# BjarkeHautop/bayesSSM

Measured on AMD Instinct MI355X. Metric: particle-steps/sec (N x T), bootstrap filter, higher is better.
Workload: dtype f64; 1 GPU; BASELINE C2: linear-Gaussian SSM, bootstrap filter, T=1000, N=1048576, SISR + systematic resampling, return_particles=FALSE, device generator; per_gpu=one independent filter replica per GPU (no data-path collective), backend=single process

## Files before the change

bayesssm_amd/csrc/fused.hip.h:

```cpp
#pragma once
#include "kernels.hip.h"

namespace bssm {

typedef unsigned long long fz_u64;
#define BSSM_RLX_AGENT __ATOMIC_RELAXED, __HIP_MEMORY_SCOPE_AGENT

constexpr int FZ_MAXB = 2 * NT;
constexpr int FZ_MINB = 256;
constexpr int FZ_KREC = 8;
constexpr int FZ_KSIDE = (int)(sizeof(SideEntry) / 4);
constexpr int FZ_NREP = 16;
constexpr int FZ_MAXSIDE = 16;
constexpr uint32_t FLAG_FUSED_BAIL = 8u, FLAG_FUSED_TIMEOUT = 16u;
constexpr uint32_t FZ_ST_DOIT = 1u, FZ_ST_DEAD = 2u, FZ_ST_STOP = 4u, FZ_ST_BAIL = 8u;
constexpr long long FZ_TIMEOUT_TICKS = 2000000ll;

struct FusedWs {
    fz_u64 e1[6][FZ_MAXB];
    fz_u64 c1[FZ_NREP][16];
    fz_u64 a1[2][FZ_MAXB];
    fz_u64 e2[FZ_KREC][FZ_MAXB];
    fz_u64 c2[FZ_NREP][16];
    fz_u64 e3[FZ_KREC][FZ_MAXB];
    fz_u64 c3[FZ_NREP][16];
    fz_u64 a3[2][FZ_MAXB];
    fz_u64 side_w[FZ_MAXB][FZ_MAXSIDE][FZ_KSIDE];
    fz_u64 side_p[FZ_MAXB][FZ_MAXSIDE][FZ_KSIDE];
    BlockRec brec_priv[2][MAXB];
    SideList side_priv[2][FZ_MAXB];
    long long stamps[2][24];
    long long startt[FZ_MAXB];
    long long endt[FZ_MAXB];
    long long waket[3][FZ_MAXB];
    long long pubt[4][FZ_MAXB];
};

#ifdef BSSM_DEV_STAMPS
#define FZ_STAMP(k) do { if (fz_stamper) g.ws->stamps[fz_row][k] = clock64(); } while (0)
#else
#define FZ_STAMP(k) do { } while (0)
#endif

__device__ __forceinline__ fz_u64 fz_gran(uint32_t tag, uint32_t v) { return ((fz_u64)tag << 32) | v; }
__device__ __forceinline__ void fz_put(fz_u64* g, uint32_t tag, uint32_t v) { __hip_atomic_store(g, fz_gran(tag, v), BSSM_RLX_AGENT); }
__device__ __forceinline__ void fz_put64(fz_u64* g, uint32_t tag, uint64_t v) { fz_put(g, tag, (uint32_t)v); fz_put(g + 1, tag, (uint32_t)(v >> 32)); }
__device__ __forceinline__ void fz_put64x(fz_u64* g, int stride, uint32_t tag, uint64_t v) { fz_put(g, tag, (uint32_t)v); fz_put(g + stride, tag, (uint32_t)(v >> 32)); }
__device__ __forceinline__ fz_u64 fz_get(const fz_u64* g) { return __hip_atomic_load(g, BSSM_RLX_AGENT); }

__device__ __forceinline__ void fz_encode(const BlockRec& br, uint32_t (&w)[FZ_KREC])
{
    const Rec& r = br.prefix;
    const long long d1 = (long long)(r.o[1] - r.o[0]), d2 = (long long)(r.o[2] - r.o[0]), d3 = (long long)(r.o[3] - r.o[0]);
    const bool fits = d1 >= -32768 && d1 <= 32767 && d2 >= -32768 && d2 <= 32767 && d3 >= -32768 && d3 <= 32767;
    const uint32_t meta = (uint32_t)(r.kind & 3) | ((uint32_t)(br.nside & 127) << 2) | ((br.tail_from < NT) ? (1u << 9) : 0u) | (fits ? 0u : (1u << 10));
    w[0] = (uint32_t)r.base; w[1] = (uint32_t)(r.base >> 32); w[2] = (uint32_t)r.o[0]; w[3] = (uint32_t)(r.o[0] >> 32);
    w[4] = ((uint32_t)d1 & 0xffffu) | (((uint32_t)d2 & 0xffffu) << 16);
    w[5] = ((uint32_t)d3 & 0xffffu) | (meta << 16);
    w[6] = (uint32_t)r.lo; w[7] = (uint32_t)r.hi;
}
__device__ __forceinline__ BlockRec fz_decode(const uint32_t (&w)[FZ_KREC], bool& unsupported)
{
    BlockRec br;
    Rec& r = br.prefix;
    r.base = mk64(w[0], w[1]); r.o[0] = mk64(w[2], w[3]);
    r.o[1] = r.o[0] + (uint64_t)(long long)(int16_t)(w[4] & 0xffffu);
    r.o[2] = r.o[0] + (uint64_t)(long long)(int16_t)(w[4] >> 16);
    r.o[3] = r.o[0] + (uint64_t)(long long)(int16_t)(w[5] & 0xffffu);
    const uint32_t meta = w[5] >> 16;
    r.kind = (int32_t)(meta & 3); r.lo = (int32_t)w[6]; r.hi = (int32_t)w[7]; r.pad = 0;
    br.nside = (int32_t)((meta >> 2) & 127);
    const bool tail = (meta >> 9) & 1u, unenc = (meta >> 10) & 1u;
    br.tail_from = tail ? 0 : NT;
    unsupported = tail || unenc || br.nside > FZ_MAXSIDE;
    return br;
}

struct FzClock { long long t0; __device__ __forceinline__ bool expired() const { return (long long)wall_clock64() - t0 > FZ_TIMEOUT_TICKS; } };

template <int NG>
__device__ __forceinline__ bool fz_wait_slot(const fz_u64* slot, uint32_t tag, const FzClock& clk, uint32_t& val)
{
    const int lane = threadIdx.x & 63;
    for (unsigned spins = 0;; spins++) {
        bool ok = true;
        if (lane < NG) { const fz_u64 x = fz_get(slot + lane); ok = (uint32_t)(x >> 32) == tag; val = (uint32_t)x; }
        if (__all(ok)) return true;
        if ((spins & 31u) == 31u && clk.expired()) return false;
        __builtin_amdgcn_s_sleep(1);
    }
}

template <int NG>
__device__ __forceinline__ bool fz_wait_words(const fz_u64* mine, uint32_t tag, const FzClock& clk, uint32_t& val)
{
    const int lane = threadIdx.x & 63;
    for (unsigned spins = 0;; spins++) {
        bool ok = true;
        if (lane < NG) { const fz_u64 x = fz_get(mine); ok = (uint32_t)(x >> 32) == tag; val = (uint32_t)x; }
        if (__all(ok)) return true;
        if ((spins & 31u) == 31u && clk.expired()) return false;
        __builtin_amdgcn_s_sleep(1);
    }
}

struct LaneTerms { double a[EL]; };
__device__ __attribute__((noinline)) void fz_block_literal(uint64_t* tin , uint64_t cin, double* terms , const LaneTerms v ,
                                                           DevState* st)
{
    const int t = threadIdx.x;
#pragma unroll
    for (int k = 0; k < EL; k++) terms[t * EL + k] = v.a[k];
    __syncthreads();
    if (t == 0) {
        double c = b2d(cin);
        for (int tt = 0; tt < NT; tt++) {
            tin[tt] = d2b(c);
            for (int k = 0; k < EL; k++) c = c + terms[tt * EL + k];
        }
        atomicAdd((unsigned long long*)&st->stat_serial_walks, 1ull);
        atomicAdd((unsigned long long*)&st->stat_literal_terms, (unsigned long long)EB);
    }
    __syncthreads();
}
__device__ __forceinline__ LaneTerms fz_lane_terms(const double (&v)[EL])
{
    LaneTerms r;
#pragma unroll
    for (int k = 0; k < EL; k++) r.a[k] = v[k];
    return r;
}

struct FusedRecSink {
    fz_u64* rec_planes;
    fz_u64* side_base;
    int bidx; uint32_t tag;
    double* terms; DevState* st;
    __device__ __forceinline__ void rec(const BlockRec& br) const
    {
        uint32_t w[FZ_KREC];
        fz_encode(br, w);
#pragma unroll
        for (int k = 0; k < FZ_KREC; k++) fz_put(rec_planes + (size_t)k * FZ_MAXB + bidx, tag, w[k]);
    }
    __device__ __forceinline__ void side(int k, const SideEntry& e) const
    {
        if (k >= FZ_MAXSIDE) return;
        uint32_t w[FZ_KSIDE];
        memcpy(w, &e, sizeof(SideEntry));
        fz_u64* dst = side_base + ((size_t)bidx * FZ_MAXSIDE + k) * FZ_KSIDE;
#pragma unroll
        for (int q = 0; q < FZ_KSIDE; q++) fz_put(dst + q, tag, w[q]);
    }
    __device__ __forceinline__ void literal(uint64_t* tin, uint64_t cin, const double (&v)[EL]) const { fz_block_literal(tin, cin, terms, fz_lane_terms(v), st); }
};

struct FusedArgs {
    const double* xin;
    long long N; int nblk;
    ModelPar par; double y; NoiseSrc ns; int trans;
    int obs_i, resample_algorithm; double threshold;
    double* ess_out; double* llh_out; int* resampled_out;
    double* w_out;
    int lim;
    int force_fallback;
    ApplyArgs a;
    FusedWs* ws; uint32_t tag;
    double* znext; uint32_t znext_call;
};

struct FusedSmem {
    double red[16]; double redq[16];
    uint32_t slot[16];
    int bail;
    double bm, bs_, bq;
};

template <int NG>
__device__ __forceinline__ bool fz_gather(const fz_u64* planes, int c0, int c1, uint32_t tag, const FzClock& clk, int* bail, uint32_t (&w0)[NG], uint32_t (&w1)[NG])
{
    const bool pair = ((c0 & 1) == 0) && (c0 < c1);
    const bool want1 = (c0 + 1 < c1);
    __amdgpu_buffer_rsrc_t rs = __builtin_amdgcn_make_buffer_rsrc((void*)const_cast<fz_u64*>(planes), 0, NG * FZ_MAXB * 8, 0x00020000);
    bool have = false;
    for (unsigned spins = 0;; spins++) {
        if (!have) {
            bool ok = true;
            if (pair) {
#pragma unroll
                for (int k = 0; k < NG; k++) {
                    const u32x4_t x = __builtin_amdgcn_raw_buffer_load_b128(rs, (k * FZ_MAXB + c0) * 8, 0, 16);
                    ok = ok && x.y == tag && (!want1 || x.w == tag); w0[k] = x.x; w1[k] = x.z;
                }
            } else {
#pragma unroll
                for (int k = 0; k < NG; k++) {
                    if (c0 < c1) { const fz_u64 x = fz_get(planes + (size_t)k * FZ_MAXB + c0); ok = ok && (uint32_t)(x >> 32) == tag; w0[k] = (uint32_t)x; }
                    if (c0 + 1 < c1) { const fz_u64 x = fz_get(planes + (size_t)k * FZ_MAXB + c0 + 1); ok = ok && (uint32_t)(x >> 32) == tag; w1[k] = (uint32_t)x; }
                }
            }
            have = ok;
        }
        if (__all(have)) return true;
        if ((spins & 15u) == 15u && clk.expired()) { *bail = 1; return false; }
        if (*(volatile int*)bail) return false;
        __builtin_amdgcn_s_sleep(1);
    }
}

__device__ __forceinline__ bool fz_fetch_sides(const fz_u64* side_base, SideList* side_priv, int b, int nside, uint32_t tag, const FzClock& clk)
{
    for (int k = 0; k < nside; k++) {
        const fz_u64* src = side_base + ((size_t)b * FZ_MAXSIDE + k) * FZ_KSIDE;
        uint32_t w[FZ_KSIDE];
        for (unsigned spins = 0;; spins++) {
            bool ok = true;
#pragma unroll
            for (int q = 0; q < FZ_KSIDE; q++) { const fz_u64 x = fz_get(src + q); ok = ok && (uint32_t)(x >> 32) == tag; w[q] = (uint32_t)x; }
            if (ok) break;
            if ((spins & 15u) == 15u && clk.expired()) return false;
            __builtin_amdgcn_s_sleep(1);
        }
        SideEntry e;
        memcpy(&e, w, sizeof(SideEntry));
        side_priv[b].e[k] = e;
    }
    return true;
}

struct FzLateSide {
    static constexpr bool active = true;
    const fz_u64* src; uint32_t tag; FzClock clk;
    __device__ __forceinline__ unsigned long long issue() const
    {
        const int lane = threadIdx.x & 63;
        static_assert(FZ_KSIDE <= 64, "one granule per lane");
        return (lane < FZ_KSIDE) ? fz_get(src + lane) : 0ull;
    }
    __device__ __forceinline__ bool finish(SideEntry* dst, unsigned long long x) const
    {
        const int lane = threadIdx.x & 63;
        for (unsigned spins = 0;; spins++) {
            const bool ok = (lane >= FZ_KSIDE) || ((uint32_t)(x >> 32) == tag);
            if (__all(ok)) {
                if (lane < FZ_KSIDE) reinterpret_cast<uint32_t*>(dst)[lane] = (uint32_t)x;
                __builtin_amdgcn_fence(__ATOMIC_RELEASE, "wavefront");
                __builtin_amdgcn_wave_barrier();
                __builtin_amdgcn_fence(__ATOMIC_ACQUIRE, "wavefront");
                return true;
            }
            if ((spins & 15u) == 15u && clk.expired()) return false;
            __builtin_amdgcn_s_sleep(1);
            if (lane < FZ_KSIDE) x = fz_get(src + lane);
        }
    }
};

template <int MODE, bool EMIT>
__device__ __forceinline__ uint64_t fz_resolve_duty(SegSmem& sm, ResolveSmem& rs, FusedSmem& fs, const FusedArgs& g, DevState* st, const FzClock& clk,
                                                    uint64_t* cin_lds , bool& bail)
{
    const int t = threadIdx.x, B = g.nblk;
    const fz_u64* planes = (MODE == MODE_W) ? &g.ws->e2[0][0] : &g.ws->e3[0][0];
    const fz_u64* sides = (MODE == MODE_W) ? &g.ws->side_w[0][0][0] : &g.ws->side_p[0][0][0];
    const int CB = (B + NT - 1) / NT;
    const int Bneed = (MODE == MODE_P) ? B - 1 : B;
    const int c0 = t * CB, c1 = (c0 + CB < Bneed) ? c0 + CB : Bneed;
    uint32_t w0[FZ_KREC], w1[FZ_KREC];
    bool ok = fz_gather<FZ_KREC>(planes, c0, c1, g.tag, clk, &fs.bail, w0, w1);
    bool unsup = false;
    BlockRec q0, q1;
    q0.prefix = rec_identity(0); q0.tail_from = NT; q0.nside = 0; q1 = q0;
    if (ok) {
        if (c0 < c1) {
            bool u; q0 = fz_decode(w0, u); unsup = unsup || u;
            if (!u && q0.nside > 0 && !(c0 == B - 1 && q0.nside == 1 && q0.tail_from >= NT)) {
#ifdef BSSM_DEV_STAMPS
                g.ws->pubt[3][20 + MODE] = c0; atomicAdd((unsigned long long*)&g.ws->pubt[3][22 + MODE], 1ull);
#endif
                ok = ok && fz_fetch_sides(sides, g.ws->side_priv[MODE], c0, q0.nside, g.tag, clk);
            }
        }
        if (c0 + 1 < c1) {
            bool u; q1 = fz_decode(w1, u); unsup = unsup || u;
            if (!u && q1.nside > 0 && !(c0 + 1 == B - 1 && q1.nside == 1 && q1.tail_from >= NT)) {
#ifdef BSSM_DEV_STAMPS
                g.ws->pubt[3][20 + MODE] = c0 + 1; atomicAdd((unsigned long long*)&g.ws->pubt[3][22 + MODE], 1ull);
#endif
                ok = ok && fz_fetch_sides(sides, g.ws->side_priv[MODE], c0 + 1, q1.nside, g.tag, clk);
            }
        }
    }
    if (unsup) atomicMax(&fs.bail, 2); else if (!ok) atomicMax(&fs.bail, 1);
    __syncthreads();
#ifdef BSSM_DEV_STAMPS
    if (t == 0) { g.ws->stamps[1][MODE == MODE_W ? 8 : 13] = clock64(); g.ws->pubt[3][8 + (MODE == MODE_W ? 1 : 2)] = (long long)wall_clock64(); }
#endif
    if (fs.bail) { bail = true; return 0ull; }
    long long lit = 0;
    const int upto = (MODE == MODE_P) ? B - 1 : B;
    FzLateSide late; late.src = sides + ((size_t)(B - 1) * FZ_MAXSIDE + 0) * FZ_KSIDE; late.tag = g.tag; late.clk = clk;
    const uint64_t fin = resolve_in_block<MODE, NT, EMIT, FzLateSide>(sm, rs, g.ws->brec_priv[MODE], g.ws->side_priv[MODE], B, upto, g.xin, g.N, 1.0, st, true, g.force_fallback, cin_lds, &lit, &q0, &q1, late);
    if (EMIT && t == 0) cin_lds[B - 1] = fin;
    if (lit >= LIT_FROM_W) fs.bail = 2;
    __syncthreads();
#ifdef BSSM_DEV_STAMPS
    if (t == 0) g.ws->stamps[1][MODE == MODE_W ? 9 : 14] = clock64();
#endif
    if (fs.bail) { bail = true; return 0ull; }
    return fin;
}

__host__ __device__ __forceinline__ int fz_resolver_block(int B) { return (5 * B) / 16; }

__device__ __forceinline__ void fz_draw_next(const FusedArgs& g, long long j0, long long N, const int prio_after = 1)
{
    if (!g.znext) return;
    __builtin_amdgcn_s_setprio(0);
#pragma unroll
    for (int i = 0; i < EL / 2; i++) {
        const long long j = j0 + 2 * i;
        if (j < N) {
            double z0, z1;
            normal_pair(g.ns.key, g.ns.purpose, g.znext_call, 0, (uint32_t)(j >> 1), z0, z1);
            if (j + 1 < N) bulk_store16<1>(g.znext + j, z0, z1);
            else g.znext[j] = z0;
        }
    }
    if (prio_after == 3) __builtin_amdgcn_s_setprio(3); else __builtin_amdgcn_s_setprio(1);
}

template <int MODEL, int KIND>
__global__ __launch_bounds__(NT) void k_obs(FusedArgs g, DevState* st)
{
    __shared__ SegSmem sm;
    __shared__ uint64_t tin[NT + 1];
    __shared__ FusedSmem fs;
    __shared__ int Tbegin;
    extern __shared__ __attribute__((aligned(16))) double dyn[];
    int* Tl = reinterpret_cast<int*>(dyn);
    double* lx = dyn + EB / 2;
    const int t = threadIdx.x, lane = t & 63, wave = t >> 6;
    const int bidx = (int)blockIdx.x, B = g.nblk;
    const bool resolver = (bidx == fz_resolver_block(B));
    if (resolver) __builtin_amdgcn_s_setprio(3); else __builtin_amdgcn_s_setprio(1);
    const bool fz_stamper = (t == 0) && (resolver || bidx == ((B > 100) ? 100 : 0)); const int fz_row = resolver ? 1 : 0; (void)fz_stamper; (void)fz_row;
    FZ_STAMP(0);
#ifdef BSSM_DEV_STAMPS
    if (t == 0) g.ws->startt[bidx] = (long long)wall_clock64();
#define FZ_PUBT(k) do { if (t == 0) g.ws->pubt[k][bidx] = (long long)wall_clock64(); } while (0)
#define FZ_GDONE(k) do { if (t == 0) g.ws->pubt[3][8 + (k)] = (long long)wall_clock64(); } while (0)
#define FZ_WAKE(k) do { if (t == 0) g.ws->waket[k][bidx] = (long long)wall_clock64(); } while (0)
#else
#define FZ_PUBT(k) do { } while (0)
#define FZ_GDONE(k) do { } while (0)
#define FZ_WAKE(k) do { } while (0)
#endif
    const long long b0 = (long long)bidx * EB, j0 = b0 + (long long)t * EL;
    const long long N = g.N;
    FzClock clk; clk.t0 = (long long)wall_clock64();
    const int s_dead = st->dead, call = st->res_calls;
    const uint32_t s_flags = st->flags;
    if (t == 0) fs.bail = 0;
    double x8[EL], l8[EL];
    if (j0 + EL <= N) {
        const double2* p = reinterpret_cast<const double2*>(g.xin + j0);
#pragma unroll
        for (int k = 0; k < EL / 2; k++) { const double2 q = p[k]; x8[2 * k] = q.x; x8[2 * k + 1] = q.y; }
    } else {
#pragma unroll
        for (int k = 0; k < EL; k++) x8[k] = (j0 + k < N) ? g.xin[j0 + k] : 0.0;
    }
    double z8[EL];
#pragma unroll
    for (int i = 0; i < EL / 2; i++) {
        const long long j = j0 + 2 * i;
        z8[2 * i] = 0.0; z8[2 * i + 1] = 0.0;
        if (g.trans && j < N) {
            if (g.ns.arr) { if (j + 1 < N) { const double2 q = *reinterpret_cast<const double2*>(g.ns.arr + j); z8[2 * i] = q.x; z8[2 * i + 1] = q.y; } else { z8[2 * i] = g.ns.arr[j]; } }
            else normal_pair(g.ns.key, g.ns.purpose, g.ns.call, 0, (uint32_t)(j >> 1), z8[2 * i], z8[2 * i + 1]);
        }
    }
    if (s_dead || s_flags) return;
#pragma unroll
    for (int i = 0; i < EL / 2; i++) {
        const long long j = j0 + 2 * i;
        if (g.trans && j < N) {
            x8[2 * i] = Model<MODEL>::transition(x8[2 * i], z8[2 * i], g.par);
            x8[2 * i + 1] = Model<MODEL>::transition(x8[2 * i + 1], z8[2 * i + 1], g.par);
        }
        l8[2 * i] = (j < N) ? r_dnorm_log(g.y, x8[2 * i], g.par.sy, g.par.log_sy) : -INFINITY;
        l8[2 * i + 1] = (j + 1 < N) ? r_dnorm_log(g.y, x8[2 * i + 1], g.par.sy, g.par.log_sy) : -INFINITY;
    }
    FZ_STAMP(1);
    double bm;
    {
        double m = l8[0];
#pragma unroll
        for (int k = 1; k < EL; k++) m = fmax(m, l8[k]);
        m = wave_max(m);
        __syncthreads();
        if (lane == 0) fs.red[wave] = m;
        __syncthreads();
        bm = fs.red[0];
#pragma unroll
        for (int i = 1; i < NWV; i++) bm = fmax(bm, fs.red[i]);
    }
    double bsum, bsq;
    {
        double sv[EL / 2], qv[EL / 2];
#pragma unroll
        for (int i = 0; i < EL / 2; i++) {
            double s_ = 0.0, q_ = 0.0;
            if (bm > -INFINITY) {
                if (l8[2 * i] > -INFINITY) { const double e = exp(l8[2 * i] - bm); s_ += e; q_ += e * e; }
                if (l8[2 * i + 1] > -INFINITY) { const double e = exp(l8[2 * i + 1] - bm); s_ += e; q_ += e * e; }
            }
            sv[i] = s_; qv[i] = q_;
        }
        static_assert(EL == 8, "four k_step pairs per lane");
        double s4 = (sv[0] + sv[1]) + (sv[2] + sv[3]), q4 = (qv[0] + qv[1]) + (qv[2] + qv[3]);
#define STEP(C) s4 = dpp_f64<C, 0xf>(0.0, s4) + s4; q4 = dpp_f64<C, 0xf>(0.0, q4) + q4;
        STEP(DPP_SHR1) STEP(DPP_SHR2) STEP(DPP_SHR4) STEP(DPP_SHR8)
#undef STEP
        __syncthreads();
        if ((lane & 15) == 15) { fs.red[4 * wave + (lane >> 4)] = s4; fs.redq[4 * wave + (lane >> 4)] = q4; }
        __syncthreads();
        double s_ = 0.0, q_ = 0.0;
#pragma unroll
        for (int i = 0; i < 16; i++) { s_ += fs.red[i]; q_ += fs.redq[i]; }
        bsum = s_; bsq = q_;
    }
    if (t < 6) {
        const uint64_t bits = d2b(t < 2 ? bm : (t < 4 ? bsum : bsq));
        fz_put(&g.ws->e1[t][bidx], g.tag, (t & 1) ? (uint32_t)(bits >> 32) : (uint32_t)bits);
    }
    FZ_STAMP(2); FZ_PUBT(0);
    if (resolver) {
        const int L = (B + NT - 1) / NT;
        const int c0 = t * L, c1 = (c0 + L < B) ? c0 + L : B;
        uint32_t w0[6], w1[6];
        const bool ok = fz_gather<6>(&g.ws->e1[0][0], c0, c1, g.tag, clk, &fs.bail, w0, w1);
        if (!ok) fs.bail = 1;
        __syncthreads();
        FZ_STAMP(3); FZ_GDONE(0);
        uint32_t status = 0;
        double M = 0.0, S = 0.0, sq = 0.0, ess1 = 0.0;
        bool book = false;
        double esv[2] = {0.0, 0.0}, pre = 0.0;
        if (!fs.bail) {
            double pmv[2], psv[2], pqv[2];
            pmv[0] = (c0 < c1) ? b2d(mk64(w0[0], w0[1])) : -INFINITY; psv[0] = (c0 < c1) ? b2d(mk64(w0[2], w0[3])) : 0.0; pqv[0] = (c0 < c1) ? b2d(mk64(w0[4], w0[5])) : 0.0;
            pmv[1] = (c0 + 1 < c1) ? b2d(mk64(w1[0], w1[1])) : -INFINITY; psv[1] = (c0 + 1 < c1) ? b2d(mk64(w1[2], w1[3])) : 0.0; pqv[1] = (c0 + 1 < c1) ? b2d(mk64(w1[4], w1[5])) : 0.0;
            M = block_max(fmax(pmv[0], pmv[1]), sm.sh4);
            const bool degenerate = (M < -1e8);
            if (degenerate) {
                if (t == 0) { st->loglike = -INFINITY; g.llh_out[g.obs_i - 1] = -INFINITY; st->dead = g.obs_i; st->do_resample = 0; }
                status = FZ_ST_DEAD;
            } else {
                double ts0 = 0.0, tq = 0.0;
#pragma unroll
                for (int k = 0; k < 2; k++) {
                    double x = 0.0;
                    if (pmv[k] > -INFINITY) { const double ex = exp(pmv[k] - M); x = psv[k] * ex; tq += pqv[k] * ex * ex; }
                    esv[k] = x; ts0 += x;
                }
                const double inc = wave_incl_sum(ts0);
                const double exc = dpp_f64<DPP_WAVE_SHR1, 0xf>(0.0, inc);
                const double wq = wave_sum(tq);
                __syncthreads();
                if (lane == 63) { sm.sh4[wave] = inc; sm.sh4[8 + wave] = wq; }
                __syncthreads();
                pre = exc;
                for (int i = 0; i < wave; i++) pre += sm.sh4[i];
                S = tree_sum<NWV>(sm.sh4);
                sq = tree_sum<NWV>(sm.sh4 + 8);
                ess1 = 1.0 / (sq / (S * S));
                const int doit = (g.resample_algorithm == 0) ? 0 : (g.resample_algorithm == 1) ? 1 : (ess1 < g.threshold);
                book = true;
                status = doit ? FZ_ST_DOIT : 0u;
                if (doit && (!(S > 0.0) || !isfinite(S) || !isfinite(M))) {
                    if (t == 0) atomicOr(&st->flags, FLAG_NONFINITE);
                    status |= FZ_ST_STOP;
                }
            }
        } else {
            status = FZ_ST_BAIL;
            if (t == 0) atomicOr(&st->flags, FLAG_FUSED_TIMEOUT);
        }
        {
            double pp = pre;
#pragma unroll
            for (int k = 0; k < 2; k++) {
                const int i = c0 + k;
                if (k < L && i < c1) fz_put64x(&g.ws->a1[0][i], FZ_MAXB, g.tag, d2b(pp / S));
                pp += esv[k];
            }
            if (t < FZ_NREP) {
                fz_u64* rep = &g.ws->c1[t][0];
                fz_put64(rep + 0, g.tag, d2b(M)); fz_put64(rep + 2, g.tag, d2b(S)); fz_put64(rep + 4, g.tag, d2b(sq)); fz_put(rep + 6, g.tag, status);
            }
        }
        if (book && t == 0) {
            const int doit = (status & FZ_ST_DOIT) ? 1 : 0;
            const double ll = st->loglike + (M + log(S) - log((double)N));
            st->loglike = ll; g.llh_out[g.obs_i - 1] = ll;
            st->do_resample = doit;
            g.ess_out[g.obs_i] = doit ? (double)N : ess1;
            if (g.resampled_out) g.resampled_out[g.obs_i - 1] = doit;
            st->ess = ess1; st->lse_max = M; st->lse_sum = S;
            if (doit) { st->cur_call = call; st->res_calls = call + 1; }
        }
    }
    if (resolver) FZ_STAMP(4);
    double M, S, a_in;
    uint32_t status;
    {
        if (wave == 0) {
            uint32_t v = 0;
            const fz_u64* src = (lane < 7) ? &g.ws->c1[bidx % FZ_NREP][lane] : &g.ws->a1[(lane - 7) & 1][bidx];
            const bool ok = fz_wait_words<9>(src, g.tag, clk, v);
            if (lane < 9) fs.slot[lane] = v;
            if (!ok && lane == 0) fs.bail = 1;
        }
        __syncthreads();
        if (fs.bail) { if (t == 0 && fs.bail == 1) atomicOr(&st->flags, FLAG_FUSED_TIMEOUT); return; }
        M = b2d(mk64(fs.slot[0], fs.slot[1])); S = b2d(mk64(fs.slot[2], fs.slot[3])); a_in = b2d(mk64(fs.slot[7], fs.slot[8]));
        status = fs.slot[6];
    }
    FZ_STAMP(5); FZ_WAKE(0);
    if (status & (FZ_ST_DEAD | FZ_ST_BAIL)) return;
    const bool doit = status & FZ_ST_DOIT;
    double v[EL];
#pragma unroll
    for (int k = 0; k < EL; k++) v[k] = (j0 + k < N) ? exp(l8[k] - M) / S : 0.0;
    if (g.w_out) {
        if (j0 + EL <= N) {
#pragma unroll
            for (int k = 0; k < EL / 2; k++) bulk_store16<BSSM_ST_W>(g.w_out + j0 + 2 * k, v[2 * k], v[2 * k + 1]);
        } else {
#pragma unroll
            for (int k = 0; k < EL; k++) if (j0 + k < N) g.w_out[j0 + k] = v[k];
        }
    }
    if (!doit) {
        double* xa = lx; double* wa = lx + EB;
        __syncthreads();
#pragma unroll
        for (int k = 0; k < EL; k++) { xa[t * EL + k] = x8[k]; wa[t * EL + k] = v[k]; }
        __syncthreads();
        double acc0 = 0.0;
#pragma unroll
        for (int r = 0; r < EL; r++) {
            const long long j = b0 + t + NT * r;
            if (j < N) { const double x0 = xa[t + NT * r]; g.a.xdst[j] = x0; acc0 += x0 * wa[t + NT * r]; }
        }
        acc0 = block_sum(acc0, sm.sh4);
        if (t == 0) g.a.se_part[bidx] = acc0;
        fz_draw_next(g, j0, N);
        return;
    }
    if (status & FZ_ST_STOP) return;
    FZ_STAMP(6);
    FusedRecSink sink; sink.bidx = bidx; sink.tag = g.tag; sink.terms = lx; sink.st = st;
    {
        BlockScan bsw;
        block_scan<MODE_W>(sm, v, a_in, g.lim, bsw);
        __syncthreads();
        sink.rec_planes = &g.ws->e2[0][0]; sink.side_base = &g.ws->side_w[0][0][0];
        block_record_tail<MODE_W, 11>(sm, tin, bsw, v, a_in, g.lim, st, 0, false, sink);
    }
    FZ_STAMP(7); FZ_PUBT(1);
    if (!resolver) fz_draw_next(g, j0, N);
    ResolveSmem& rs = *reinterpret_cast<ResolveSmem*>(dyn);
    uint64_t* cin_lds = reinterpret_cast<uint64_t*>(reinterpret_cast<char*>(dyn) + ((sizeof(ResolveSmem) + 15) / 16) * 16);
    if (resolver) {
        __syncthreads();
        bool bail = false;
        const uint64_t fin = fz_resolve_duty<MODE_W, false>(sm, rs, fs, g, st, clk, nullptr, bail);
        uint32_t stw = 0;
        if (bail) { stw = FZ_ST_BAIL; if (t == 0) atomicOr(&st->flags, fs.bail == 1 ? FLAG_FUSED_TIMEOUT : FLAG_FUSED_BAIL); }
        else {
            const double tot = b2d(fin);
            if (t == 0) {
                st->total_bits = fin;
                if (tot == 0.0) atomicOr(&st->flags, FLAG_ZERO_SUM);
                if (!isfinite(tot)) atomicOr(&st->flags, FLAG_NONFINITE);
            }
            if (tot == 0.0 || !isfinite(tot)) stw = FZ_ST_STOP;
        }
        if (t < FZ_NREP) { fz_put64(&g.ws->c2[t][0], g.tag, fin); fz_put(&g.ws->c2[t][2], g.tag, stw); }
        fz_draw_next(g, j0, N);
        FZ_STAMP(10);
    }
    double total;
    {
        __syncthreads();
        if (wave == 0) {
            uint32_t vv = 0;
            const bool ok = fz_wait_slot<3>(&g.ws->c2[bidx % FZ_NREP][0], g.tag, clk, vv);
            if (lane < 3) fs.slot[lane] = vv;
            if (!ok && lane == 0) fs.bail = 1;
        }
        __syncthreads();
        if (fs.bail) { if (t == 0 && fs.bail == 1) atomicOr(&st->flags, FLAG_FUSED_TIMEOUT); return; }
        if (fs.slot[2] & (FZ_ST_BAIL | FZ_ST_STOP)) return;
        total = b2d(mk64(fs.slot[0], fs.slot[1]));
    }
    FZ_STAMP(11); FZ_WAKE(1);
    const double a_in_p = a_in / total;
#pragma unroll
    for (int k = 0; k < EL; k++) v[k] = v[k] / total;
    BlockScan bs;
#ifdef BSSM_DEV_STAMPS
    const bool xstamper = (t == 0 && bidx == B / 4);
    const int xdbg = 99;
    if (xstamper) st->stamps[2][10] = clock64();
#else
    const bool xstamper = false; const int xdbg = 0;
#endif
    block_scan<MODE_P>(sm, v, a_in_p, g.lim, bs);
    __syncthreads();
#ifdef BSSM_DEV_STAMPS
    if (xstamper) st->stamps[2][11] = clock64();
#endif
    sink.rec_planes = &g.ws->e3[0][0]; sink.side_base = &g.ws->side_p[0][0][0];
    block_record_tail<MODE_P, 3>(sm, tin, bs, v, a_in_p, g.lim, st, xdbg, xstamper, sink);
#ifdef BSSM_DEV_STAMPS
    if (xstamper) { st->stamps[2][9] = clock64(); st->stamps[2][8] = bs.nb; }
#endif
    FZ_STAMP(12); FZ_PUBT(2);
    uint64_t cinb = 0;
    if (resolver) {
        __syncthreads();
        bool bail = false;
        (void)fz_resolve_duty<MODE_P, true>(sm, rs, fs, g, st, clk, cin_lds, bail);
        uint32_t stp = 0;
        if (bail) { stp = FZ_ST_BAIL; if (t == 0) atomicOr(&st->flags, fs.bail == 1 ? FLAG_FUSED_TIMEOUT : FLAG_FUSED_BAIL); }
        for (int b = t; b < B; b += NT) fz_put64x(&g.ws->a3[0][b], FZ_MAXB, g.tag, bail ? 0ull : cin_lds[b]);
        if (t < FZ_NREP) fz_put(&g.ws->c3[t][0], g.tag, stp);
        FZ_STAMP(15);
        if (bail) return;
        cinb = cin_lds[bidx];
        __syncthreads();
    } else {
        __syncthreads();
        if (wave == 0) {
            uint32_t vv = 0;
            const fz_u64* src = (lane < 2) ? &g.ws->a3[lane & 1][bidx] : &g.ws->c3[bidx % FZ_NREP][0];
            const bool ok = fz_wait_words<3>(src, g.tag, clk, vv);
            if (lane < 3) fs.slot[lane] = vv;
            if (!ok && lane == 0) fs.bail = 1;
        }
        __syncthreads();
        if (fs.bail) { if (t == 0 && fs.bail == 1) atomicOr(&st->flags, FLAG_FUSED_TIMEOUT); return; }
        if (fs.slot[2] & FZ_ST_BAIL) return;
        cinb = mk64(fs.slot[0], fs.slot[1]);
    }
    FZ_STAMP(16); FZ_WAKE(2);
    uint64_t ent;
    {
        const bool good = block_resolve<MODE_P>(sm, bs, cinb, g.lim, nullptr, 0, total, b0, ent);
        if (!good) { fz_block_literal(tin, cinb, lx, fz_lane_terms(v), st); ent = tin[t]; }
    }
    FZ_STAMP(17);
    double xs0[EL], xs1[EL], axs[EL];
    __syncthreads();
#pragma unroll
    for (int k = 0; k < EL; k++) lx[t * EL + k] = x8[k];
    __syncthreads();
    {
        const int ebase = wave * (64 * EL) + lane;
#pragma unroll
        for (int k = 0; k < EL; k++) { xs0[k] = lx[ebase + 64 * k]; xs1[k] = 0.0; axs[k] = 0.0; }
    }
    if (t == 0) sm.big = 0;
    UniformSrc us;
    us.arr = g.a.u_base ? g.a.u_base + (long long)call * g.a.u_stride : nullptr;
    us.key = g.a.key; us.call = (uint32_t)call;
    const double Usys = (KIND == 1) ? us(0) : 0.0;
    __syncthreads();
    apply_tail<KIND, false, CAPX, false>(sm, Tl, Tbegin, bidx, B, g.a, st, g.a.nstage ? lx + EB : nullptr, g.a.nstage, v, ent, xs0, xs1, axs, call, us, Usys, 0, false, lx);
    FZ_STAMP(18);
#ifdef BSSM_DEV_STAMPS
    if (t == 0) g.ws->pubt[3][32 + (bidx & 255)] = 0;
    __syncthreads();
    if (t == 0) g.ws->endt[bidx] = (long long)wall_clock64();
#endif
}

constexpr size_t FZ_DYN_LDS = (size_t)EB * sizeof(int) + (size_t)(EB + CAPX) * sizeof(double);
static_assert(((sizeof(ResolveSmem) + 15) / 16) * 16 + FZ_MAXB * sizeof(uint64_t) <= FZ_DYN_LDS, "the resolver's scratch borrows the workers' staging area");

}
```

bayesssm_amd/csrc/kernels.hip.h:

```cpp
#pragma once
#include <hip/hip_runtime.h>
#include <stdint.h>
#include <math.h>
#include "seqsum.h"
#include "rng.h"

namespace bssm {

#ifndef BSSM_NT
#define BSSM_NT 256
#endif
#ifndef BSSM_EL
#define BSSM_EL 8
#endif
constexpr int NT = BSSM_NT;
constexpr int EL = BSSM_EL;
constexpr int NWV = NT / 64;
static_assert(NT * EL == 2048 && (NT == 256 || NT == 512) , "a scan workgroup covers 2048 terms with 4 or 8 waves");
constexpr int EB = NT * EL;
constexpr int MAXB = 2048;

typedef double v2d_nt __attribute__((ext_vector_type(2)));
#ifndef BSSM_ST_W
#define BSSM_ST_W 0
// ... 1231 lines not shown
        a_in = sm.bcast;
        BSSM_STAMP(st, dbg, 2, 8, stamper);
        if (f.xw) {
#pragma unroll
            for (int k = 0; k < EL; k++) l8[k] = r_dnorm_log(f.yw, l8[k], f.syw, f.lsyw);
        }
#pragma unroll
        for (int k = 0; k < EL; k++) v[k] = (j0 + k < nw) ? exp(l8[k] - M) / S : 0.0;
        if (j0 + EL <= nw || (LIT && j0 < nw)) {
            double2* p2 = reinterpret_cast<double2*>(f.w_out + j0);
#pragma unroll
            for (int k = 0; k < EL / 2; k++) bulk_store16<BSSM_ST_W>(reinterpret_cast<double*>(p2 + k), v[2 * k], v[2 * k + 1]);
        } else {
#pragma unroll
            for (int k = 0; k < EL; k++) if (j0 + k < nw) f.w_out[j0 + k] = v[k];
        }
        if (!doit) return;
        if (!(S > 0.0) || !isfinite(S) || !isfinite(M)) {
            if (t == 0) atomicOr(&st->flags, FLAG_NONFINITE);
            return;
        }
        BSSM_STAMP(st, dbg, 2, 9, stamper);
    } else {
#pragma unroll
        for (int k = 0; k < EL; k++) v[k] = (MODE == MODE_P) ? vraw[k] / total : vraw[k];
        a_in = a_in_pre;
    }
    BSSM_STAMP(st, dbg, 2, 1, stamper && v[0] >= 0.0);
    if (LIT) {
        __syncthreads();
        block_literal_terms(tin, FROM_LW ? f.w_out : w, (int)nw);
        if (t == NT - 1) { BlockRec br; br.prefix = rec_abs(tin[NT]); br.tail_from = NT; br.nside = 0; store_brec(brec, bidx, br, bstride); }
        return;
    }
    BlockScan bs;
    block_scan<MODE>(sm, v, a_in, lim, bs);
    __syncthreads();
    BSSM_STAMP(st, dbg, 2, FROM_LW ? 10 : 2, stamper);
    GlobalRecSink<MODE> sink; sink.brec = brec; sink.sides = side; sink.bidx = bidx; sink.bstride = bstride;
    sink.w = w; sink.nw = nw; sink.total = total; sink.b0 = b0; sink.st = st;
    if constexpr (FROM_LW) block_record_tail<MODE, 11>(sm, tin, bs, v, a_in, lim, st, dbg, stamper, sink);
    else block_record_tail<MODE, 3>(sm, tin, bs, v, a_in, lim, st, dbg, stamper, sink);
}


constexpr long long LIT_FROM_W = 1ll << 40;
template <int MODE>
__device__ __forceinline__ uint64_t block_out_exact_body(const BlockRec& br, const SideList* __restrict__ side, const double* __restrict__ w,
                                                         long long nw, double total, long long b, uint64_t in, long long& lit)
{
    bool ok = true;
    uint64_t o = rec_step(br.prefix, in, ok);
    const long long e0 = b * EB, e1 = (e0 + EB < nw) ? e0 + EB : nw;
    if (!ok) {
        lit += ((e1 > e0) ? e1 - e0 : 0) + LIT_FROM_W;
        return literal_run<MODE>(w, nw, total, e0, e1, in);
    }
    if (br.nside > 0) {
        const SideEntry* se = side[b].e;
        for (int k = 0; k < br.nside; k++) {
            const SideEntry e = se[k];
            bool ok2 = true;
            uint64_t o2 = rec_step(e.leaf, o, ok2);
            if (!ok2) {
                double c = b2d(o);
#pragma unroll
                for (int q = 0; q < EL; q++) c = c + e.terms[q];
                o2 = d2b(c);
                lit += EL;
            }
            o = o2;
            if (e.pad) {
                const int64_t diff = (int64_t)(o - e.post_base);
                if (diff < (int64_t)e.lo || diff > (int64_t)e.hi) {
                    const long long j0 = e0 + (long long)(e.lane + 1) * EL;
                    if (j0 < e1) { lit += e1 - j0 + LIT_FROM_W; o = literal_run<MODE>(w, nw, total, j0, e1, o); }
                    return o;
                }
                Pure p; p.d0 = e.d0; p.d1 = e.d1;
                o = pure_step(p, o);
            }
        }
        return o;
    }
    if (br.tail_from >= NT) return o;
    const long long j0 = e0 + (long long)br.tail_from * EL;
    if (j0 >= e1) return o;
    lit += e1 - j0 + LIT_FROM_W;
    return literal_run<MODE>(w, nw, total, j0, e1, o);
}

struct OutLit { uint64_t out; long long lit; };
template <int MODE>
__device__ __attribute__((noinline)) OutLit block_out_exact_nl(const BlockRec* br, const SideList* side, const double* w,
                                                               long long nw, double total, long long b, uint64_t in)
{
    OutLit r; r.lit = 0;
    r.out = block_out_exact_body<MODE>(*br, side, w, nw, total, b, in, r.lit);
    return r;
}
template <int MODE>
__device__ __forceinline__ uint64_t block_out_exact(const BlockRec& br, const SideList* __restrict__ side, const double* __restrict__ w,
                                                    long long nw, double total, long long b, uint64_t in, long long& lit)
{
    const OutLit r = block_out_exact_nl<MODE>(&br, side, w, nw, total, b, in);
    lit += r.lit;
    return r.out;
}

struct ResolveSmem {
    BlockRec bnd[64];
    Pure ex[64];
    int ebidx[64];
    uint64_t sout[65];
    __attribute__((aligned(16))) SideEntry sideC[64];
    uint64_t result;
    int fail;
};

struct LaneRun { Pure p; long long wlo, whi; uint64_t base; int any; };

__device__ __forceinline__ void run_reset(LaneRun& r) { r.p.d0 = 0; r.p.d1 = 0; r.wlo = -(1ll << 40); r.whi = (1ll << 40); r.base = 0; r.any = 0; }
__device__ __forceinline__ void run_fold(LaneRun& r, const Rec& pr)
{
    if (!r.any) { r.base = pr.base; r.any = 1; }
    const long long m0 = (long long)(r.base + (uint64_t)r.p.d0 - pr.base);
    const long long m1 = (long long)(r.base + 1 + (uint64_t)r.p.d1 - pr.base);
    const long long mmin = m0 < m1 ? m0 : m1, mmax = m0 > m1 ? m0 : m1;
    const long long lo = (long long)pr.lo - mmin + 2, hi = (long long)pr.hi - mmax - 2;
    r.wlo = lo > r.wlo ? lo : r.wlo; r.whi = hi < r.whi ? hi : r.whi;
    Pure q; q.d0 = (int64_t)(pr.o[0] - pr.base); q.d1 = (int64_t)(pr.o[1] - (pr.base + 1));
    r.p = pure_compose(r.p, q);
}
__device__ __forceinline__ void run_merge(LaneRun& r, const LaneRun& q)
{
    if (!q.any) return;
    if (!r.any) { r = q; return; }
    const long long m0 = (long long)(r.base + (uint64_t)r.p.d0 - q.base);
    const long long m1 = (long long)(r.base + 1 + (uint64_t)r.p.d1 - q.base);
    const long long mmin = m0 < m1 ? m0 : m1, mmax = m0 > m1 ? m0 : m1;
    const long long lo = q.wlo - mmin + 2, hi = q.whi - mmax - 2;
    r.wlo = lo > r.wlo ? lo : r.wlo; r.whi = hi < r.whi ? hi : r.whi;
    r.p = pure_compose(r.p, q.p);
}
__device__ __forceinline__ bool run_ok(const LaneRun& r, uint64_t ent)
{
    if (!r.any) return true;
    const long long diff = (long long)(ent - r.base);
    return diff >= r.wlo && diff <= r.whi;
}

struct NoLateSide {
    static constexpr bool active = false;
    __device__ __forceinline__ unsigned long long issue() const { return 0ull; }
    __device__ __forceinline__ bool finish(SideEntry*, unsigned long long) const { return true; }
};
template <int MODE, int NTX = NT, bool EMIT = false, class LateSide = NoLateSide>
__device__ __forceinline__ uint64_t resolve_in_block(SegSmem& sm, ResolveSmem& rs, const BlockRec* __restrict__ brec,
                                                     const SideList* __restrict__ side, const int B, const int upto,
                                                     const double* __restrict__ w, long long nw, double total, DevState* st,
                                                     const bool count_stats, const int ff ,
                                                     uint64_t* __restrict__ cin_out = nullptr,
                                                     long long* lit_out = nullptr ,
                                                     const BlockRec* pre0 = nullptr, const BlockRec* pre1 = nullptr ,
                                                     const LateSide late = LateSide())
{
    const int t = threadIdx.x;
    if (upto <= 0) return 0ull;
    const int dbg = st->debug_stop; (void)dbg;
    const bool stamper = (t == 0 && (EMIT || blockIdx.x == 100)); (void)stamper;
    BSSM_STAMP(st, dbg, MODE, 0, stamper);
    const int CB = (B + NTX - 1) / NTX;
    const int c0 = t * CB, c1 = (c0 + CB < upto) ? c0 + CB : upto;
    BlockRec r0, r1;
    r0.prefix = rec_identity(0); r0.tail_from = NT; r0.nside = 0; r1 = r0;
    if (c0 < c1) r0 = pre0 ? *pre0 : load_brec(brec, c0);
    if (c0 + 1 < c1) r1 = pre1 ? *pre1 : load_brec(brec, c0 + 1);
    if (t == 0) { rs.sout[0] = 0; rs.fail = 0; }
    if (!LateSide::active && upto == B && t >= NTX - (int)(sizeof(SideEntry) / 16)) {
        const int q = t - (NTX - (int)(sizeof(SideEntry) / 16));
        reinterpret_cast<uint4*>(&rs.sideC[63])[q] = reinterpret_cast<const uint4*>(&side[upto - 1].e[0])[q];
    }
    LaneRun head, tail;
    run_reset(head); run_reset(tail);
    const bool x0 = (c0 < c1) && !(r0.prefix.kind == REC_PURE && r0.tail_from >= NT && r0.nside == 0);
    const bool x1 = (c0 + 1 < c1) && !(r1.prefix.kind == REC_PURE && r1.tail_from >= NT && r1.nside == 0);
    if (c0 < c1 && !x0) run_fold(head, r0.prefix);
    if (c0 + 1 < c1 && !x1) { if (x0) run_fold(tail, r1.prefix); else run_fold(head, r1.prefix); }
    const int nent = (x0 ? 1 : 0) + (x1 ? 1 : 0);
    int ent_before, E;
    const Pure carry = seg_excl_scan_tail<NTX / 64>(sm, nent ? tail.p : head.p, nent > 0, nent, ent_before, E);
    const bool fits = (E <= 64);
    if (fits && nent) {
        int slot = ent_before;
        if (x0) { rs.bnd[slot] = r0; rs.ebidx[slot] = c0; rs.ex[slot] = carry; slot++; }
        if (x1) { rs.bnd[slot] = r1; rs.ebidx[slot] = c0 + 1; if (x0) { rs.ex[slot].d0 = 0; rs.ex[slot].d1 = 0; } else rs.ex[slot] = pure_compose(carry, head.p); }
    }
    __syncthreads();
    BSSM_STAMP(st, dbg, MODE, 2, stamper);
    long long lit = 0;
    if (fits && t < 64) {
        const int lane = t;
        const bool have = lane < E;
        unsigned long long late_v = 0ull;
        if constexpr (LateSide::active) { if (upto == B) late_v = late.issue(); }
        int bidx = -1;
        Pure ex; ex.d0 = 0; ex.d1 = 0;
        Rec pr = rec_identity(0);
        int nside = 0;
        bool slow = false;
        if (have) {
            bidx = rs.ebidx[lane]; ex = rs.ex[lane];
            pr = rs.bnd[lane].prefix; nside = rs.bnd[lane].nside;
            slow = (nside > 1) || (rs.bnd[lane].tail_from < NT);
            if (nside == 1 && !slow && !(upto == B && bidx == B - 1 && lane < 63)) {
                const uint4* sp = reinterpret_cast<const uint4*>(&side[bidx].e[0]);
                uint4* dp = reinterpret_cast<uint4*>(&rs.sideC[lane]);
#pragma unroll
                for (int q = 0; q < (int)(sizeof(SideEntry) / 16); q++) dp[q] = sp[q];
            }
        }
        const int side_slot = (upto == B && bidx == B - 1 && lane < 63) ? 63 : lane;
        uint64_t sw = 0, my_out = 0, my_s0 = 0;
        const bool special = have && (slow || nside == 1);
        const StepFn fn = stepfn_build(ex, pr);
        const WalkFn wfn = walkfn_from(fn, have && !special);
        BSSM_STAMP(st, dbg, MODE, 3, stamper && wfn.sh >= 0);
        const int j0 = walk_chain_regs(wfn, E, sw, my_s0, my_out);
        BSSM_STAMP(st, dbg, MODE, 4, stamper && sw != 1);
        if constexpr (LateSide::active) {
            if (upto == B && E > 0 && E <= 64) {
                const int lb = __builtin_amdgcn_readlane(bidx, E - 1), ln = __builtin_amdgcn_readlane(nside, E - 1), ls = __builtin_amdgcn_readlane((int)slow, E - 1);
                if (lb == B - 1 && ln == 1 && !ls) { if (!late.finish(&rs.sideC[63], late_v)) lit += LIT_FROM_W; }
            }
        }
        for (int j = j0; j < E; j++) {
            bool ok;
            uint64_t o = stepfn_apply(fn, sw, ok);
            const uint64_t e = pure_step(ex, sw);
            if (lane == j && (special || !ok)) {
                bool done = false;
                if (!slow && ok && nside == 1 && !ff_on<MODE>(ff, FF_GENERAL_LINK)) {
                    const SideEntry& se = rs.sideC[side_slot];
                    bool ok2 = true;
                    uint64_t o2 = rec_step(se.leaf, o, ok2);
                    if (!ok2) {
                        double c = b2d(o);
#pragma unroll
                        for (int q = 0; q < EL; q++) c = c + se.terms[q];
                        o2 = d2b(c);
                    }
                    done = true;
                    if (se.pad) {
                        const int64_t diff = (int64_t)(o2 - se.post_base);
                        if (diff < (int64_t)se.lo || diff > (int64_t)se.hi) done = false;
                        else { Pure pp; pp.d0 = se.d0; pp.d1 = se.d1; o2 = pure_step(pp, o2); }
                    }
                    if (done) o = o2;
                }
                if (!done) {
                    if (LateSide::active && upto == B && bidx == B - 1 && nside == 1 && !slow) lit += LIT_FROM_W;
                    else o = block_out_exact<MODE>(rs.bnd[lane], side, w, nw, total, bidx, e, lit);
                }
            }
            if (lane == j) my_out = o;
            sw = readlane_u64(o, j);
        }
        BSSM_STAMP(st, dbg, MODE, 5, stamper && sw != 1);
        if (have) rs.sout[lane + 1] = my_out;
    }
    if ((!fits || ff_on<MODE>(ff, FF_SERIAL_WALK)) && t == 0) rs.fail = 1;
    __syncthreads();
    BSSM_STAMP(st, dbg, MODE, 6, stamper);
    if (fits && c0 < c1) {
        const uint64_t ent = pure_step(carry, rs.sout[ent_before]);
        bool ok = true;
        uint64_t end;
        if (nent == 0) { ok = run_ok(head, ent); end = pure_step(head.p, ent); }
        else {
            ok = run_ok(head, ent);
            const uint64_t after = rs.sout[ent_before + nent];
            ok = ok && run_ok(tail, after);
            end = pure_step(tail.p, after);
        }
        if (!ok) rs.fail = 1;
        if (c1 == upto) rs.result = end;
        if constexpr (EMIT) {
            cin_out[c0] = ent;
            if (c0 + 1 < c1) {
                LaneRun h0; run_reset(h0); run_fold(h0, r0.prefix);
                cin_out[c0 + 1] = x0 ? rs.sout[ent_before + 1] : pure_step(h0.p, ent);
            }
        }
    }
    __syncthreads();
    if (rs.fail) {
        if (pre0) {
            if (c0 < c1) store_brec(const_cast<BlockRec*>(brec), c0, r0);
            if (c0 + 1 < c1) store_brec(const_cast<BlockRec*>(brec), c0 + 1, r1);
            __syncthreads();
        }
        if (t == 0) {
            uint64_t sf = 0;
            for (int b = 0; b < upto; b++) {
                const BlockRec r = load_brec(brec, b);
                if (EMIT) cin_out[b] = sf;
                if (LateSide::active && upto == B && b == B - 1 && r.nside == 1 && r.tail_from >= NT) { lit += LIT_FROM_W; break; }
                sf = block_out_exact<MODE>(r, side, w, nw, total, b, sf, lit);
            }
            rs.result = sf;
            if (count_stats) atomicAdd((unsigned long long*)&st->stat_serial_walks, 1ull);
        }
        __syncthreads();
    }
    if (lit && count_stats) atomicAdd((unsigned long long*)&st->stat_literal_terms, (unsigned long long)(lit & (LIT_FROM_W - 1)));
    if (lit_out) *lit_out = lit;
    BSSM_STAMP(st, dbg, MODE, 7, stamper);
#ifdef BSSM_DEV_STAMPS
    if ((dbg == 99 || dbg == 98) && stamper) { st->stamps[MODE][8] = E; st->stamps[MODE][9] = upto; }
#endif
    return rs.result;
}

template <int MODE>
struct InResolve {
    static constexpr bool active = true;
    SegSmem* sm; ResolveSmem* rs; const BlockRec* brec; const SideList* side; int B, upto;
    const double* w; long long nw; double total; DevState* st; bool stats; int ff;
    __device__ __forceinline__ uint64_t operator()() const { return resolve_in_block<MODE>(*sm, *rs, brec, side, B, upto, w, nw, total, st, stats, ff); }
};

template <int MODE, bool FROM_LW, bool INRES = false>
__global__ __launch_bounds__(NT) void k_local(const double* __restrict__ w, long long nw, const double* __restrict__ ain,
                                              int lim, BlockRec* __restrict__ brec, SideList* __restrict__ side, DevState* st,
                                              FromLw f, const BlockRec* __restrict__ prev_brec, const SideList* __restrict__ prev_side,
                                              double* __restrict__ ain_p_out, int boff, int nblk_g)
{
    __shared__ SegSmem sm;
    __shared__ uint64_t tin[NT];
    __shared__ double es[1];
    const int bidx = (int)blockIdx.x + boff, nblk = nblk_g ? nblk_g : (int)gridDim.x;
    if constexpr (INRES) {
        static_assert(!INRES || (MODE == MODE_P && !FROM_LW), "only the cumsum pass resolves the pass before it");
        __shared__ ResolveSmem rs;
        InResolve<MODE_W> pro; pro.sm = &sm; pro.rs = &rs; pro.brec = prev_brec; pro.side = prev_side; pro.B = nblk; pro.upto = nblk;
        pro.w = w; pro.nw = nw; pro.total = 1.0; pro.st = st; pro.stats = (bidx == 0); pro.ff = st->force_fallback;
        local_block<MODE, FROM_LW, MAXB, false, InResolve<MODE_W>>(sm, tin, es, bidx, nblk, w, nw, ain, lim, brec, side, st, f, pro, ain_p_out);
    } else {
        (void)prev_brec; (void)prev_side; (void)ain_p_out;
        local_block<MODE, FROM_LW, MAXB>(sm, tin, es, bidx, nblk, w, nw, ain, lim, brec, side, st, f);
    }
}

constexpr int NTR = 1024;
constexpr int SIDE_CACHE = 12;

template <int MODE>
__global__ __launch_bounds__(NTR) void k_resolve(const double* __restrict__ w, long long nw, int B,
                                                 const BlockRec* __restrict__ brec, const SideList* __restrict__ side,
                                                 uint64_t* __restrict__ cin,
                                                 const double* __restrict__ ain_w, double* __restrict__ ain_p, DevState* st)
{
    extern __shared__ __attribute__((aligned(16))) char smraw[];
    BlockRec* br = reinterpret_cast<BlockRec*>(smraw);
    __shared__ SegSmem sm;
    __shared__ uint64_t final_state;
    __shared__ __attribute__((aligned(16))) SideEntry sideC[64];
    const int t = threadIdx.x;
    const int s_dead = st->dead, s_do = st->do_resample, dbg0 = st->debug_stop; (void)dbg0;
    const int ff = st->force_fallback;
    const uint32_t s_flags = st->flags;
    const uint64_t s_total = st->total_bits;
    BSSM_STAMP(st, dbg0, MODE, 0, t == 0);
    BSSM_STAMP(st, dbg0, MODE, 1, t == 0);
    if (t >= NTR - (int)(sizeof(SideEntry) / 16)) {
        const int q = t - (NTR - (int)(sizeof(SideEntry) / 16));
        reinterpret_cast<uint4*>(&sideC[63])[q] = reinterpret_cast<const uint4*>(&side[B - 1].e[0])[q];
    }
    {
        const uint4* src = reinterpret_cast<const uint4*>(brec);
        uint4* dst = reinterpret_cast<uint4*>(smraw);
        const int n16 = B * (int)(sizeof(BlockRec) / 16);
        for (int i = t; i < n16; i += NTR) dst[i] = src[(size_t)(i & 3) * BREC_STRIDE + (i >> 2)];
    }
    if (t == 0) sm.fail = 0;
    __syncthreads();
    if (s_dead || s_flags || !s_do) return;
    BSSM_STAMP(st, dbg0, MODE, 2, t == 0);
    const double total = (MODE == MODE_P) ? b2d(s_total) : 1.0;
    const int CB = (B + NTR - 1) / NTR;
    const int c0 = t * CB, c1 = (c0 + CB < B) ? c0 + CB : B;
    bool isb = false;
    Pure comp; comp.d0 = 0; comp.d1 = 0;
    long long wlo = -(1ll << 40), whi = (1ll << 40);
    uint64_t cbase = 0;
    for (int b = c0; b < c1; b++) {
        const BlockRec& r = br[b];
        if (r.prefix.kind != REC_PURE || r.tail_from < NT || r.nside > 0) { isb = true; break; }
        if (b == c0) cbase = r.prefix.base;
        const long long m0 = (long long)(cbase + (uint64_t)comp.d0 - r.prefix.base);
        const long long m1 = (long long)(cbase + 1 + (uint64_t)comp.d1 - r.prefix.base);
        const long long mmin = m0 < m1 ? m0 : m1, mmax = m0 > m1 ? m0 : m1;
        const long long lo = (long long)r.prefix.lo - mmin + 2, hi = (long long)r.prefix.hi - mmax - 2;
        wlo = lo > wlo ? lo : wlo; whi = hi < whi ? hi : whi;
        Pure p; p.d0 = (int64_t)(r.prefix.o[0] - r.prefix.base); p.d1 = (int64_t)(r.prefix.o[1] - (r.prefix.base + 1));
        comp = pure_compose(comp, p);
    }
    if (c0 >= B) { isb = false; comp.d0 = comp.d1 = 0; }
    BSSM_STAMP(st, dbg0, MODE, 3, t == 0);
    int seg, nb; Pure lastseg;
    const Pure exc = seg_excl_scan<NTR / 64>(sm, comp, isb, seg, nb, lastseg);
    if (isb && seg < MAXBND) { sm.bnd_excl[seg] = exc; sm.bnd_lane[seg] = t; }
    __syncthreads();
    BSSM_STAMP(st, dbg0, MODE, 4, t == 0);
    long long lit = 0;
    const int nent = nb * CB;
#ifdef BSSM_DEV_STAMPS
    if (dbg0 == 99 && t == 0) { st->stamps[MODE][8] = nb; st->stamps[MODE][9] = B; }
#endif
    if (t < 64) {
        const int lane = t;
        const bool fits = (nb <= MAXBND) && (nent <= 64) && !ff_on<MODE>(ff, FF_SERIAL_WALK);
        const bool have = fits && lane < nent;
        const int k = have ? lane / CB : 0;
        int bidx = -1;
        Pure ex; ex.d0 = 0; ex.d1 = 0;
        if (have) {
            bidx = sm.bnd_lane[k] * CB + (lane % CB);
            if (bidx >= B) bidx = -1;
            if (lane % CB == 0) ex = sm.bnd_excl[k];
        }
        Rec pr = rec_identity(0);
        int nside = 0;
        bool slow = false;
        if (bidx >= 0) {
            pr = br[bidx].prefix; nside = br[bidx].nside;
            slow = (nside > 1) || (br[bidx].tail_from < NT);
            if (nside == 1 && !slow && fits && !(bidx == B - 1 && lane < 63)) {
                const uint4* sp = reinterpret_cast<const uint4*>(&side[bidx].e[0]);
                uint4* dp = reinterpret_cast<uint4*>(&sideC[lane]);
#pragma unroll
                for (int q = 0; q < (int)(sizeof(SideEntry) / 16); q++) dp[q] = sp[q];
            }
        }
        if (!fits) { if (lane == 0) sm.fail = 1; }
        else {
            uint64_t s = 0, my_in = 0, my_out = 0;
            const bool special = (bidx >= 0) && (slow || nside == 1);
            const StepFn fn = stepfn_build(ex, pr);
// ... 1149 lines not shown
```

Measured before the change: 22.07 billion particle-steps/s.

## Publish weight-sum total early from resolver wave before block-wide finalize

In the fused resolver for the weight mode, the wave that completes the segmented scan computes the final total directly and publishes it to the c2 replicas before the block synchronizes and runs the end-of-resolve checks. Waiting blocks can then proceed with resampling sooner, taking the cross-block handoff latency off the critical path. If the block later fails validation after an early publish, it signals a bail through the a3/c3 channels instead of recomputing serially. This adds a plausibility gate (total between 0.5 and 2) and a more complex failure protocol that could be wrong when the early value disagrees with the exact path.

```diff
diff --git a/bayesssm_amd/csrc/fused.hip.h b/bayesssm_amd/csrc/fused.hip.h
--- a/bayesssm_amd/csrc/fused.hip.h
+++ b/bayesssm_amd/csrc/fused.hip.h
@@ -173,7 +173,9 @@
     double red[16]; double redq[16];
     uint32_t slot[16];
     int bail;
+    int early;
     double bm, bs_, bq;
+    Pure fin_run;
 };
 
 template <int NG>
@@ -228,9 +230,33 @@
     return true;
 }
 
+template <bool EARLY>
 struct FzLateSide {
     static constexpr bool active = true;
+    static constexpr bool early = EARLY;
     const fz_u64* src; uint32_t tag; FzClock clk;
+    fz_u64* early_dst;
+    FusedSmem* fs;
+#ifdef BSSM_DEV_STAMPS
+    long long* early_stamp;
+#endif
+    __device__ __forceinline__ void early_run(const Pure& p) const { if (EARLY) fs->fin_run = p; }
+    __device__ __forceinline__ bool early_done() const { return EARLY && fs->early; }
+    __device__ __forceinline__ void early_publish(uint64_t s) const
+    {
+        if (!EARLY) return;
+        const int lane = threadIdx.x & 63;
+        const uint64_t fin = pure_step(fs->fin_run, s);
+        const double tot = b2d(fin);
+        if (!(tot > 0.5 && tot < 2.0)) return;
+        if (lane < FZ_NREP) { fz_u64* rep = early_dst + lane * 16; fz_put64(rep, tag, fin); fz_put(rep + 2, tag, 0u); }
+        if (lane == 0) {
+            fs->early = 1;
+#ifdef BSSM_DEV_STAMPS
+            *early_stamp = clock64();
+#endif
+        }
+    }
     __device__ __forceinline__ unsigned long long issue() const
     {
         const int lane = threadIdx.x & 63;
@@ -299,8 +325,13 @@
     if (fs.bail) { bail = true; return 0ull; }
     long long lit = 0;
     const int upto = (MODE == MODE_P) ? B - 1 : B;
-    FzLateSide late; late.src = sides + ((size_t)(B - 1) * FZ_MAXSIDE + 0) * FZ_KSIDE; late.tag = g.tag; late.clk = clk;
-    const uint64_t fin = resolve_in_block<MODE, NT, EMIT, FzLateSide>(sm, rs, g.ws->brec_priv[MODE], g.ws->side_priv[MODE], B, upto, g.xin, g.N, 1.0, st, true, g.force_fallback, cin_lds, &lit, &q0, &q1, late);
+    typedef FzLateSide<MODE == MODE_W> Late;
+    Late late; late.src = sides + ((size_t)(B - 1) * FZ_MAXSIDE + 0) * FZ_KSIDE; late.tag = g.tag; late.clk = clk;
+    late.early_dst = &g.ws->c2[0][0]; late.fs = &fs;
+#ifdef BSSM_DEV_STAMPS
+    late.early_stamp = &g.ws->stamps[1][19];
+#endif
+    const uint64_t fin = resolve_in_block<MODE, NT, EMIT, Late>(sm, rs, g.ws->brec_priv[MODE], g.ws->side_priv[MODE], B, upto, g.xin, g.N, 1.0, st, true, g.force_fallback, cin_lds, &lit, &q0, &q1, late);
     if (EMIT && t == 0) cin_lds[B - 1] = fin;
     if (lit >= LIT_FROM_W) fs.bail = 2;
     __syncthreads();
@@ -361,7 +392,10 @@
     FzClock clk; clk.t0 = (long long)wall_clock64();
     const int s_dead = st->dead, call = st->res_calls;
     const uint32_t s_flags = st->flags;
-    if (t == 0) fs.bail = 0;
+    if (t == 0) { fs.bail = 0; fs.early = 0; }
+#ifdef BSSM_DEV_STAMPS
+    if (resolver && t == 0) g.ws->stamps[1][19] = 0;
+#endif
     double x8[EL], l8[EL];
     if (j0 + EL <= N) {
         const double2* p = reinterpret_cast<const double2*>(g.xin + j0);
@@ -579,17 +613,21 @@
         bool bail = false;
         const uint64_t fin = fz_resolve_duty<MODE_W, false>(sm, rs, fs, g, st, clk, nullptr, bail);
         uint32_t stw = 0;
+        const bool early = fs.early;
         if (bail) { stw = FZ_ST_BAIL; if (t == 0) atomicOr(&st->flags, fs.bail == 1 ? FLAG_FUSED_TIMEOUT : FLAG_FUSED_BAIL); }
-        else {
-            const double tot = b2d(fin);
-            if (t == 0) {
-                st->total_bits = fin;
-                if (tot == 0.0) atomicOr(&st->flags, FLAG_ZERO_SUM);
-                if (!isfinite(tot)) atomicOr(&st->flags, FLAG_NONFINITE);
-            }
-            if (tot == 0.0 || !isfinite(tot)) stw = FZ_ST_STOP;
-        }
-        if (t < FZ_NREP) { fz_put64(&g.ws->c2[t][0], g.tag, fin); fz_put(&g.ws->c2[t][2], g.tag, stw); }
+        if (bail && early) {
+            for (int b = t; b < B; b += NT) fz_put64x(&g.ws->a3[0][b], FZ_MAXB, g.tag, 0ull);
+            if (t < FZ_NREP) fz_put(&g.ws->c3[t][0], g.tag, FZ_ST_BAIL);
+            return;
+        }
+        const double tot = b2d(fin);
+        if (!bail && (tot == 0.0 || !isfinite(tot))) stw = FZ_ST_STOP;
+        if (!early && t < FZ_NREP) { fz_put64(&g.ws->c2[t][0], g.tag, fin); fz_put(&g.ws->c2[t][2], g.tag, stw); }
+        if (!bail && t == 0) {
+            st->total_bits = fin;
+            if (tot == 0.0) atomicOr(&st->flags, FLAG_ZERO_SUM);
+            if (!isfinite(tot)) atomicOr(&st->flags, FLAG_NONFINITE);
+        }
         fz_draw_next(g, j0, N);
         FZ_STAMP(10);
     }
diff --git a/bayesssm_amd/csrc/kernels.hip.h b/bayesssm_amd/csrc/kernels.hip.h
--- a/bayesssm_amd/csrc/kernels.hip.h
+++ b/bayesssm_amd/csrc/kernels.hip.h
@@ -1407,8 +1407,12 @@
 
 struct NoLateSide {
     static constexpr bool active = false;
+    static constexpr bool early = false;
     __device__ __forceinline__ unsigned long long issue() const { return 0ull; }
     __device__ __forceinline__ bool finish(SideEntry*, unsigned long long) const { return true; }
+    __device__ __forceinline__ void early_run(const Pure&) const { }
+    __device__ __forceinline__ void early_publish(uint64_t) const { }
+    __device__ __forceinline__ bool early_done() const { return false; }
 };
 template <int MODE, int NTX = NT, bool EMIT = false, class LateSide = NoLateSide>
 __device__ __forceinline__ uint64_t resolve_in_block(SegSmem& sm, ResolveSmem& rs, const BlockRec* __restrict__ brec,
@@ -1451,6 +1455,7 @@
         if (x0) { rs.bnd[slot] = r0; rs.ebidx[slot] = c0; rs.ex[slot] = carry; slot++; }
         if (x1) { rs.bnd[slot] = r1; rs.ebidx[slot] = c0 + 1; if (x0) { rs.ex[slot].d0 = 0; rs.ex[slot].d1 = 0; } else rs.ex[slot] = pure_compose(carry, head.p); }
     }
+    if constexpr (LateSide::early) { if (fits && c0 < c1 && c1 == upto) late.early_run(nent ? tail.p : pure_compose(carry, head.p)); }
     __syncthreads();
     BSSM_STAMP(st, dbg, MODE, 2, stamper);
     long long lit = 0;
@@ -1523,6 +1528,7 @@
         }
         BSSM_STAMP(st, dbg, MODE, 5, stamper && sw != 1);
         if (have) rs.sout[lane + 1] = my_out;
+        if constexpr (LateSide::early) { if (!__any(lit >= LIT_FROM_W)) late.early_publish(sw); }
     }
     if ((!fits || ff_on<MODE>(ff, FF_SERIAL_WALK)) && t == 0) rs.fail = 1;
     __syncthreads();
@@ -1549,7 +1555,9 @@
         }
     }
     __syncthreads();
-    if (rs.fail) {
+    if (LateSide::early && rs.fail && late.early_done()) {
+        if (t == 0) lit += LIT_FROM_W;
+    } else if (rs.fail) {
         if (pre0) {
             if (c0 < c1) store_brec(const_cast<BlockRec*>(brec), c0, r0);
             if (c0 + 1 < c1) store_brec(const_cast<BlockRec*>(brec), c0 + 1, r1);
```

Measured after the change: 22.39 billion particle-steps/s, median of 6. 1.4% higher.
